# thedeemon/jsplayer

Measured on AMD Instinct MI355X. Metric: decoded Mpixels/sec at 1920x1080 (MSVideo1 + ScreenPressor), 1/2/4/8 GPUs, higher is better.
Workload: dtype u8

## Files before the change

jsplayer_amd/csrc/msv1.h:

```cpp
#pragma once
#include <cstddef>
#include <cstdint>
#include <vector>

#include <hip/hip_runtime.h>

namespace jsp {

constexpr uint32_t MSV1_DESC_SKIP = 0xFFFFFFFFu;
constexpr uint32_t MSV1_DESC_UNTOUCHED = 0xFFFFFFFEu;

struct Msv1FrameArgs {
    int32_t* dst;
    const int32_t* prev;
    uint32_t* signif;
    uint32_t stream_end;
    uint32_t desc_base;
    uint32_t cmp_row_lo;
    uint32_t pad;
};

constexpr uint32_t MSV1_FRAME_USES_PREV = 1u;
constexpr uint32_t MSV1_FRAME_NOOP = 2u;

// ... 30 lines not shown
constexpr uint32_t MSV1_INFO_END_MARKER = 1u;
constexpr uint32_t MSV1_INFO_S1 = 2u;
struct Msv1FrameInfo {
    uint32_t n_coded;
    uint32_t n_skip_codes;
    uint32_t total_blocks;
    uint32_t flags;
    uint32_t consumed;
    uint32_t pad[3];
};
uint32_t msv1_parse_tile_bytes();
uint32_t msv1_small_tile_bytes();
void msv1_launch_parse(const Msv1Geometry& geo, const uint8_t* d_stream, const Msv1ParseFrame* d_frames, int nframes,
                       const uint32_t* d_tile_frame, int ntiles, int max_tiles_per_frame, uint32_t* d_tile_tab,
                       uint32_t* d_tile_entry, uint32_t* d_tile_block0, uint32_t* d_desc, Msv1FrameInfo* d_info,
                       int insignificant_blocks, hipStream_t stream);

constexpr uint32_t MSV1_TILE_SKIP = 1u;
struct alignas(16) Msv1TileRec {
    uint32_t byte0;
    uint32_t frame_end;
    uint32_t data_end;
    uint32_t k;
    uint32_t first_tile;
    uint32_t ntiles;
    uint32_t cmp_row_lo;
    uint32_t flags;
    int32_t* dst;
    const int32_t* prev;
    uint32_t* signif;
    uint64_t pad;
};
static_assert(sizeof(Msv1TileRec) == 64, "one record = 64 bytes");
constexpr size_t MSV1_AGG_PUBLISHED = 9;
constexpr size_t MSV1_AGG_LAB_CLOCKS = 8;
constexpr size_t MSV1_SYNC_BYTES = 2 * sizeof(uint32_t) + 64;

struct Msv1FusedBatch {
    const uint8_t* stream = nullptr;
    const Msv1TileRec* recs = nullptr;
    const int32_t* palette = nullptr;
    unsigned long long* agg = nullptr;
    uint32_t epoch = 0;
    uint32_t tile0 = 0;
    int ntiles = 0;
    uint32_t* fault = nullptr;
    uint32_t agg_tiles = 0;
};
void msv1_launch_fused_pixels(const Msv1Geometry& geo, const Msv1FusedBatch& batch, hipStream_t stream);
void msv1_launch_fused_tables(const Msv1Geometry& geo, const Msv1FusedBatch& batch, hipStream_t stream);

constexpr uint32_t MSV1_ASYNC_SHORT = 1u;
constexpr uint32_t MSV1_ASYNC_S1 = 2u;
constexpr uint32_t MSV1_ASYNC_END = 4u;
constexpr uint32_t MSV1_ASYNC_SKIPCODE = 8u;
constexpr uint32_t MSV1_ASYNC_STUCK = 16u;
struct Msv1AsyncInfo {
    uint32_t flags;
    uint32_t signif;
    uint32_t fault;
    uint32_t arrived;
    uint32_t finished;
    uint32_t verdict;
    uint32_t pad[2];
};
constexpr uint32_t MSV1_VERDICT_GO = 1u, MSV1_VERDICT_VETO = 2u;
constexpr uint32_t MSV1_LAB_DEAF = 0x80000000u;
// ... 51 lines not shown
```

jsplayer_amd/csrc/msv1_codec.cpp:

```cpp
#include <algorithm>
#include <atomic>
#include <memory>
#include <exception>
#include <thread>
#include <unordered_set>

#include "codec.h"
#include "msv1.h"
#include "msv1_seek.h"
#include <msv1_fused_hooks.h>

namespace jsp {
namespace {

inline uint32_t next_epoch(uint32_t& e) { if (++e == 0) ++e; return e; }

inline size_t agg_bytes(size_t tiles) { return sizeof(unsigned long long) * (MSV1_AGG_PUBLISHED + MSV1_AGG_LAB_CLOCKS) * std::max<size_t>(tiles, 1); }

inline Msv1TileRec tile_rec(uint32_t beg, uint32_t even_end, uint32_t data_end, uint32_t k, uint32_t tile_bytes, uint32_t first_tile, uint32_t ntiles,
                            int32_t* dst, const int32_t* prev, uint32_t* signif, uint32_t cmp_row_lo, uint32_t flags) {
    Msv1TileRec r{};
    r.byte0 = beg + k * tile_bytes;
    r.frame_end = even_end;
    r.data_end = data_end;
// ... 125 lines not shown
                          d_tile_tab.as<uint32_t>(), d_tile_entry.as<uint32_t>(), d_tile_block0.as<uint32_t>(), d_desc.as<uint32_t>(), d_info.as<Msv1FrameInfo>(),
                          insignificant_blocks, stream);
    }

    void decode(hipStream_t stream) override {
        if (nframes == 0) return;
        last_stream = stream;
        const bool replay = gpu_parse && decoded && needs_desc;
        const bool run_ahead = side != nullptr && gpu_parse && needs_desc && ntiles_emit > 0;
        if (replay) {
            if (run_ahead && ahead_valid) JSP_HIP(hipStreamWaitEvent(stream, ev_tables, 0));
            else launch_table_parse(cur_set, stream);
        }
        const uint32_t* tables = replay ? wide_tables(cur_set) : d_desc.as<const uint32_t>();
        if (run_ahead && decoded) {
            try {
                make_set(cur_set ^ 1, stream);
            } catch (const std::exception&) {
                (void)hipGetLastError();
                sets[cur_set ^ 1].drop();
                side = nullptr;
            }
        }
        if (run_ahead && decoded && side) {
            if (!ev_fork) JSP_HIP(hipEventCreateWithFlags(&ev_fork, hipEventDisableTiming));
            if (!ev_tables) JSP_HIP(hipEventCreateWithFlags(&ev_tables, hipEventDisableTiming));
            JSP_HIP(hipEventRecord(ev_fork, stream));
            JSP_HIP(hipStreamWaitEvent(side, ev_fork, 0));
            launch_table_parse(cur_set ^ 1, side);
            JSP_HIP(hipEventRecord(ev_tables, side));
        }
        launch_groups(tables, true, stream);
        if (any_fused || needs_desc)
            JSP_HIP(hipMemcpyAsync(h_fault.p, d_sync.p, sizeof(uint32_t), hipMemcpyDeviceToHost, stream));
        ++clock_launches;
        if (run_ahead && decoded && side) { cur_set ^= 1; ahead_valid = true; }
        decoded = true;
    }
    void plan_launches(const std::vector<jsp_frame_in>& frames, const StagePlan& plan) {
        const auto& attr = plan.attr;
        const int nf = nframes;
        int i = 0;
        while (i < nf) {
            if (attr[i].special) { groups.push_back({i, 1, attr[i].edge, false, false}); ++i; continue; }
            int j = i;
            bool any_dep = false;
            while (j < nf && !attr[j].special) { any_dep |= attr[j].dependent; ++j; }
            std::unordered_set<const void*> seen;
            if (any_dep && vec_ok) {
                bool edge = false;
                for (int k = i; k < j; ++k) edge |= attr[k].edge;
                groups.push_back({i, j - i, edge, true, false});
            } else {
                bool closed = true;
                for (int k = i; k < j; ++k) {
                    const bool writes = !attr[k].noop;
                    const bool fusable = gpu_parse && vec_ok && !attr[k].dependent && !attr[k].noop && !plan.h_pf[k].host_parsed;
                    if (attr[k].dependent || closed || (writes && seen.count(frames[k].dst)) || groups.back().fused != fusable) {
                        groups.push_back({k, 1, attr[k].edge, false, fusable});
                        seen.clear();
                        closed = attr[k].dependent;
                    } else {
                        groups.back().count++;
                    }
                    if (writes) seen.insert(frames[k].dst);
                }
            }
// ... 19 lines not shown
            uint64_t written = 0, prev_reads = 0, sbytes = 0;
            bool uses_prev = false, gpu_table = false;
            for (int k = g.first; k < g.first + g.count; ++k) {
                if (!plan.attr[k].noop) written += (uint64_t)geo.nblocks;
                uses_prev |= (h_frames[k].pad & MSV1_FRAME_USES_PREV) != 0;
                if (h_frames[k].pad & MSV1_FRAME_USES_PREV) prev_reads += (uint64_t)geo.nblocks;
                sbytes += plan.frame_stream[k];
                gpu_table |= gpu_parse && !plan.h_pf[k].host_parsed;
            }
            moved += sbytes + 64 * written;
            if (g.fused) {
                any_fused = true;
                note_kernel("msv1_fused_kernel");
            } else {
                needs_desc |= gpu_table;
                moved += table_bytes_per_frame * g.count +
                         64 * (g.temporal ? (uses_prev ? (uint64_t)geo.nblocks : 0) : prev_reads);
                note_kernel(g.temporal ? "msv1_blocks_temporal_kernel" : "msv1_blocks_kernel");
            }
            if (g.edge_compare) note_kernel("msv1_edge_compare_kernel");
        }
        if (needs_desc) {
            moved += info.stream_bytes + table_bytes_per_frame * nf;
            if (!any_fused) kernels = "msv1_fused_kernel" + (kernels.empty() ? std::string() : " + " + kernels);
        }
        info.moved_bytes = moved;
        info.kernel_launches = groups.size() + (needs_desc ? 1 : 0);
    }

    void build_tile_records(const std::vector<jsp_frame_in>& frames, const StagePlan& plan, bool scrub_tables, hipStream_t stream) {
        if (!any_fused && !needs_desc) return;
        d_agg.reserve(agg_bytes((size_t)ntiles));
        d_sync.reserve(MSV1_SYNC_BYTES);
        h_fault.reserve(sizeof(uint32_t));
        *h_fault.as<uint32_t>() = 0;
        epoch = 0;
        build_pixel_records(plan, stream);
        if (needs_desc) build_table_records(frames, plan, scrub_tables, stream);
        JSP_HIP(hipMemsetAsync(d_agg.p, 0, agg_bytes((size_t)ntiles), stream));
        JSP_HIP(hipMemsetAsync(d_sync.p, 0, MSV1_SYNC_BYTES, stream));
    }
    void build_pixel_records(const StagePlan& plan, hipStream_t stream) {
        const int nf = nframes;
        const Msv1ParseFrame* h_pf = plan.h_pf;
        const auto* h_frames = this->h_frames.as<const Msv1FrameArgs>();
        h_recs.reserve(sizeof(Msv1TileRec) * (size_t)std::max(ntiles, 1));
        d_recs.reserve(sizeof(Msv1TileRec) * (size_t)std::max(ntiles, 1));
        auto* recs = h_recs.as<Msv1TileRec>();
        std::vector<uint32_t> nt16((size_t)nf);
        for (int i = 0; i < nf; ++i) {
            nt16[i] = h_pf[i].ntiles;
            for (uint32_t k = 0; k < h_pf[i].ntiles; ++k)
                recs[h_pf[i].first_tile + k] = tile_rec(h_pf[i].beg, h_pf[i].end, geo.bits == 16 ? h_pf[i].end : h_frames[i].stream_end, k, msv1_parse_tile_bytes(),
                                                        h_pf[i].first_tile, h_pf[i].ntiles, h_frames[i].dst, h_frames[i].prev, h_frames[i].signif,
                                                        h_frames[i].cmp_row_lo, h_pf[i].host_parsed ? MSV1_TILE_SKIP : 0u);
        }
        auto tile_major = [&](int f0, int f1) {
            if (f1 - f0 < 2) return;
            const uint32_t t0 = h_pf[f0].first_tile, t1 = h_pf[f1 - 1].first_tile + h_pf[f1 - 1].ntiles;
            const std::vector<Msv1TileRec> tmp(recs + t0, recs + t1);
            uint32_t o = t0;
            staggered_tile_order(f0, f1, nt16, MSV1_TILE_STAGGER, [&](int i, uint32_t k) { recs[o++] = tmp[h_pf[i].first_tile - t0 + k]; });
        };
        for (const auto& g : groups)
            if (g.fused) tile_major(g.first, g.first + g.count);
        JSP_HIP(hipMemcpyAsync(d_recs.p, recs, sizeof(Msv1TileRec) * (size_t)ntiles, hipMemcpyHostToDevice, stream));
    }
    void build_table_records(const std::vector<jsp_frame_in>& frames, const StagePlan& plan, bool scrub_tables, hipStream_t stream) {
        const int nf = nframes;
        const Msv1ParseFrame* h_pf = plan.h_pf;
        const auto* h_frames = this->h_frames.as<const Msv1FrameArgs>();
        const size_t nblk = (size_t)std::max(geo.nblocks, 1);
        const uint32_t tile8 = msv1_small_tile_bytes();
// ... 27 lines not shown
    }

    void launch_groups(const uint32_t* tables, bool fused, hipStream_t stream) {
        if (need_signif) JSP_HIP(hipMemsetAsync(d_signif.p, 0, sizeof(uint32_t) * nframes, stream));
        const auto* frames = d_frames.as<const Msv1FrameArgs>();
        for (const Group& g : groups) {
            if (g.fused && fused) {
                const auto* pf = h_pframes.as<const Msv1ParseFrame>();
                const uint32_t tile0 = pf[g.first].first_tile;
                const Msv1ParseFrame& last = pf[g.first + g.count - 1];
                msv1_launch_fused_pixels(geo, fused_batch(d_recs, d_agg, ntiles, tile0, (int)(last.first_tile + last.ntiles - tile0)), stream);
            } else if (g.temporal) {
                msv1_launch_blocks_temporal(geo, d_stream.as<const uint8_t>(), tables, frames + g.first, g.count, d_palette, stream);
            } else {
                msv1_launch_blocks(geo, d_stream.as<const uint8_t>(), tables, frames + g.first, g.count, d_palette, vec_ok, stream);
            }
            if (g.edge_compare) msv1_launch_edge_compare(geo, frames + g.first, g.count, stream);
        }
        JSP_HIP(hipGetLastError());
        if (need_signif) JSP_HIP(hipMemcpyAsync(h_signif.p, d_signif.p, sizeof(uint32_t) * nframes, hipMemcpyDeviceToHost, stream));
    }
    int clock_launches = 0;
    void after_sync() override {
        if (kFusedClocks && clock_launches) {
            std::vector<unsigned long long> c((size_t)ntiles * MSV1_AGG_LAB_CLOCKS);
            unsigned long long* dev = d_agg.as<unsigned long long>() + (size_t)ntiles * MSV1_AGG_PUBLISHED;
            JSP_HIP(hipMemcpy(c.data(), dev, c.size() * 8, hipMemcpyDeviceToHost));
            JSP_HIP(hipMemset(dev, 0, c.size() * 8));
            unsigned long long h[8] = {0, 0, 0, 0, 0, 0, 0, 0};
            for (size_t i = 0; i < c.size(); ++i) h[i & 7] += c[i];
            const unsigned long long n = (unsigned long long)ntiles * clock_launches;
            std::fprintf(stderr, "fused clocks per tile (cycles; %d tiles x %d launches): load %llu | tables+trees %llu | look-back %llu | down %llu | replay %llu | decode %llu\n",
                         ntiles, clock_launches, h[0] / n, h[1] / n, h[2] / n, h[3] / n, h[4] / n, h[5] / n);
        }
        clock_launches = 0;
        if ((any_fused || needs_desc) && (*h_fault.as<const uint32_t>() || inject_fault)) {
            inject_fault = false;
            ++fallback_runs;
            if (fallback_total) ++*fallback_total;
            note_kernel("msv1_parse_tiles (look-back fallback)");
            *h_fault.as<uint32_t>() = 0;
            hipStream_t stream = last_stream;
            quiesce_side();
            JSP_HIP(hipMemsetAsync(d_sync.p, 0, MSV1_SYNC_BYTES, stream));
            launch_parse(stream);
            launch_groups(d_desc.as<const uint32_t>(), false, stream);
            JSP_HIP(hipStreamSynchronize(stream));
        }
    }
    hipStream_t last_stream = nullptr;
    bool inject_fault = false;
    int fallback_runs = 0;
    std::shared_ptr<std::atomic<long long>> fallback_total;
};

struct Msv1AsyncStaged : jsp_staged {
    Msv1AsyncStaged() { verdict_pending = true; }
    Msv1Geometry geo{};
    Msv1AsyncShared shared;
    int ntiles = 0;
    size_t nbytes = 0;
    bool have_prev = false, compare = false, key = false;
    bool key_compare = false;
    DeviceBuffer d_stream, d_meta, d_agg;
    PinnedBuffer h_stream, h_meta, h_info;
    uint32_t epoch = 0;
    size_t agg_tiles = 0;
    bool merged = false;
    bool deaf = false;
    Msv1TileRec rec{};
    DeviceBuffer d_report;
    uint32_t want = 0;
    const uint8_t* src_dev = nullptr;
    hipEvent_t uploaded = nullptr;
    bool dma = false;
    bool stale_before = false;
    const void* full_dev_before = nullptr;
    size_t full_dev_bytes_before = 0;
    ~Msv1AsyncStaged() override { if (uploaded) (void)hipEventDestroy(uploaded); }

    Msv1AsyncInfo* d_info() const {
        if (merged) return d_report.as<Msv1AsyncInfo>();
        return reinterpret_cast<Msv1AsyncInfo*>(d_meta.as<uint8_t>() + sizeof(Msv1TileRec) * (size_t)ntiles);
    }
    uint32_t bad_mask() const { return MSV1_ASYNC_SHORT | MSV1_ASYNC_END | MSV1_ASYNC_STUCK | (have_prev ? 0u : MSV1_ASYNC_SKIPCODE) | (deaf ? MSV1_LAB_DEAF : 0u); }
    Msv1GroupFrame group_frame(hipStream_t stream) {
// ... 17 lines not shown
    void decode(hipStream_t stream) override {
        if (merged) { decode_with({}, stream); return; }
        Msv1FusedPass pass;
        pass.stream = d_stream.as<const uint8_t>();  pass.recs = d_meta.as<const Msv1TileRec>();  pass.ntiles = ntiles;
        pass.agg = d_agg.as<unsigned long long>();   pass.info = d_info();  pass.bad_mask = bad_mask();  pass.shared = shared;
        pass.epoch = next_epoch(epoch);
        msv1_launch_fused_scout(geo, pass, stream);
        pass.epoch = next_epoch(epoch);
        msv1_launch_fused_decode(geo, pass, stream);
        JSP_HIP(hipGetLastError());
        JSP_HIP(hipMemcpyAsync(h_info.p, pass.info, sizeof(Msv1AsyncInfo), hipMemcpyDeviceToHost, stream));
        decoded = true;
    }
};

std::atomic<int> g_async_streams{0};
constexpr int kDmaStreams = 3;

struct Msv1Codec : jsp_codec {
    Msv1Geometry geo{};
    size_t size_of_just_skips = 0;
    int insignificant_blocks = 0;
    bool insign_lines_set = false;
    int insign_lines = 0;
    std::vector<uint8_t> block_changes;
    std::vector<uint8_t> palette_bytes;
    int32_t palette[256];
    DeviceBuffer d_palette;
    bool opt_gpu_parse = true;
    bool opt_scrub_tables = false;
    bool opt_inject_fault = false;
    bool opt_inject_deaf = false;
    std::shared_ptr<std::atomic<long long>> lookback_fallbacks = std::make_shared<std::atomic<long long>>(0);
    long long counter(const char* name) override {
        if (std::strcmp(name, "prefetched_frames") == 0) return prefetched_frames;
        if (std::strcmp(name, "paired_frames") == 0) return paired_frames;
        if (std::strcmp(name, "host_parsed_frames") == 0) return host_parsed_frames;
        if (std::strcmp(name, "msv1_block_changes") == 0) {
            std::vector<uint8_t> rows;
            try {
                if (!msv1_block_changes_now(this, rows)) return -1;
            } catch (const std::exception&) {
                return -1;
            }
            long long m = 0;
            for (size_t r = 0; r < rows.size() && r < 62; ++r) m |= (long long)(rows[r] != 0) << r;
            return m;
        }
        return std::strcmp(name, "lookback_fallbacks") == 0 ? lookback_fallbacks->load() : -1;
    }
    bool opt_async_merged = true, opt_async_dma = true, opt_async_auto = true;
    bool counted_async = false;
    hipStream_t up_stream = nullptr;
    struct UpRange {
        const uint8_t* host = nullptr;
        size_t bytes = 0, skew = 0;
        DeviceBuffer dev;
        hipEvent_t up = nullptr, last_use = nullptr;
        bool waited = false;
        hipStream_t waited_on = nullptr;
        bool used = false;
    };
    static constexpr int kRanges = 4;
    UpRange ranges[kRanges];
    unsigned range_next = 0;
    hipStream_t prefetch_stream = nullptr;
    long long prefetched_frames = 0;
    long long host_parsed_frames = 0;
    int prefetch(const void* host, size_t n) override {
        if (!host || n == 0) {
            for (UpRange& r : ranges) { r.host = nullptr; r.bytes = 0; }
            return 0;
        }
        if (!opt_gpu_parse) return 0;
        launch_held();
        UpRange& r = ranges[range_next++ % kRanges];
        r.host = nullptr;
        r.bytes = 0;
        if (!prefetch_stream) JSP_HIP(hipStreamCreateWithFlags(&prefetch_stream, hipStreamNonBlocking));
        if (!r.up) {
            JSP_HIP(hipEventCreateWithFlags(&r.up, hipEventDisableTiming));
// ... 207 lines not shown
            block_changes_stale = false;
        }
        msv1_parse(geo, src, n, prev_dev != nullptr, size_of_just_skips, insignificant_blocks, base, desc,
                   block_changes, pr);
    }

    struct Prescan { bool sync_path, changes; };
    Prescan prescan(const uint8_t* src, size_t n) const {
        if (n < 2 || (geo.bits == 16 && n < size_of_just_skips)) return {true, false};
        long covered = 0;
        for (size_t si = 0; si + 1 < n && covered < geo.nblocks; si += 2) {
            const unsigned a = src[si], b = src[si + 1];
            if (geo.bits == 8 && a == 0 && b == 0) return {true, false};
            if ((b & 0xFC) != 0x84) return {false, true};
            const long cnt = (long)(((b - 0x84) << 8) + a);
            if (cnt == 0) return {true, false};
            covered += cnt;
        }
        return {covered < geo.nblocks, false};
    }

    bool sync_staging(const jsp_frame_in& f, const Prescan& ps) const {
        const bool aligned = (X & 3) == 0 && !(reinterpret_cast<uintptr_t>(f.dst) & 15) && !(reinterpret_cast<uintptr_t>(prev_dev) & 15);
        return !opt_gpu_parse || !aligned || (Y & 3) || ps.sync_path || geo.nblocks <= 0 || geo.nblocks >= (1 << 20) ||
               f.n + msv1_parse_tile_bytes() > 0xFFFFFFF0u || (geo.bits == 8 && !d_palette.p);
    }
    bool async_settle_first(const jsp_frame_in& f) override { return sync_staging(f, prescan(f.src, f.n)); }
    bool sync_through_async() const override { return opt_gpu_parse; }

    void reserve_async_buffers(Msv1AsyncStaged& st, int nt, size_t tile_bytes) {
        st.d_stream.reserve((size_t)nt * tile_bytes + 64);
        st.h_info.reserve(sizeof(Msv1AsyncInfo));
        if ((size_t)nt > st.agg_tiles) {
            st.d_agg.reserve(sizeof(unsigned long long) * 9 * (size_t)nt);
            st.agg_tiles = st.d_agg.cap / (sizeof(unsigned long long) * 9);
            JSP_HIP(hipMemsetAsync(st.d_agg.p, 0, st.d_agg.cap, stream));
        }
        if (st.merged && !st.d_report.p) {
            st.d_report.reserve(sizeof(Msv1AsyncInfo));
            JSP_HIP(hipMemsetAsync(st.d_report.p, 0, sizeof(Msv1AsyncInfo), stream));
            st.want = 0;
        }
        if (!st.merged) {
            const size_t meta_bytes = sizeof(Msv1TileRec) * (size_t)nt + sizeof(Msv1AsyncInfo);
            st.d_meta.reserve(meta_bytes);
            st.h_meta.reserve(meta_bytes);
        }
    }

    struct FrameBytes { const void* up; const uint8_t* up_dev; UpRange* range; };
    FrameBytes frame_bytes(const jsp_frame_in& f, Msv1AsyncStaged& st) {
        hipPointerAttribute_t attr{};
        UpRange* range = range_of(f.src, f.n);
        if (range) {
            if (!range->waited || range->waited_on != stream) {
                JSP_HIP(hipStreamWaitEvent(stream, range->up, 0));
                range->waited = true;
                range->waited_on = stream;
            }
            range->used = true;
            ++prefetched_frames;
            return {f.src, range->dev.as<const uint8_t>() + range->skew + (f.src - range->host), range};
        }
        if (hipPointerGetAttributes(&attr, f.src) == hipSuccess && attr.type == hipMemoryTypeHost)
            return {f.src, static_cast<const uint8_t*>(attr.devicePointer ? attr.devicePointer : f.src), nullptr};
        (void)hipGetLastError();
        st.h_stream.reserve(f.n + 16);
        std::memcpy(st.h_stream.p, f.src, f.n);
// ... 150 lines not shown
        st->build_tile_records(frames, plan, opt_scrub_tables, stream);
        st->info.host_stage_ms = now_ms() - t0 - plan.gpu_parse_ms;
        final_uploads(*st, plan);
        st->info.h2d_ms = plan.h2d_ms;
        st->info.device_parse_ms = plan.gpu_parse_ms;
        guard.release();
        return st;
    }

    void upload(void* d, const void* h, size_t bytes) {
        if (bytes) JSP_HIP(hipMemcpyAsync(d, h, bytes, hipMemcpyHostToDevice, stream));
    }

    void reset_batch(Msv1Staged& st, int nf) {
        st.quiesce_side();
        st.drop_sets();
        st.side = nullptr;
        if (opt_parse_ahead) {
            if (!side_stream) JSP_HIP(hipStreamCreateWithFlags(&side_stream, hipStreamNonBlocking));
            st.side = side_stream;
        }
        st.geo = geo;
        st.nframes = nf;
        st.decoded = false;
        st.groups.clear();
        st.status.assign(nf, JSP_ZERO_STATE);
        st.adopted.assign(nf, 0);
        st.significant.assign(nf, 0);
        st.info = jsp_staged_info{};
        st.why.clear();
        st.insignificant_blocks = insignificant_blocks;
        st.inject_fault = opt_inject_fault;
        st.fallback_total = lookback_fallbacks;
        st.gpu_parse = opt_gpu_parse && geo.nblocks > 0 && geo.nblocks < (1 << 20);
        if (geo.bits == 8 && !d_palette.p) {
            d_palette.reserve(sizeof palette);
            JSP_HIP(hipMemcpy(d_palette.p, palette, sizeof palette, hipMemcpyHostToDevice));
        }
        st.d_palette = d_palette.as<const int32_t>();
    }

    void lay_out_and_gather(const std::vector<jsp_frame_in>& frames, Msv1Staged& st, StagePlan& plan) {
        const int nf = (int)frames.size();
        const size_t nblk = (size_t)std::max(geo.nblocks, 1);
        plan.beg.resize(nf);
        const size_t frame_align = st.gpu_parse ? (size_t)msv1_parse_tile_bytes() : 16;
        for (int i = 0; i < nf; ++i) {
            plan.beg[i] = plan.total_stream;
            plan.total_stream += (frames[i].n + frame_align - 1) / frame_align * frame_align;
        }
        if (plan.total_stream + 64 > 0xFFFFFFF0u) throw std::runtime_error("batch stream exceeds 4 GiB");
        plan.in_pinned.assign(nf, 0);
        size_t gather_bytes = 0;
        for (int i = 0; i < nf; ++i) {
            if (st.gpu_parse && frames[i].n >= 4096) {
                hipPointerAttribute_t attr{};
                if (hipPointerGetAttributes(&attr, frames[i].src) == hipSuccess && attr.type == hipMemoryTypeHost) plan.in_pinned[i] = 1;
                else (void)hipGetLastError();
            }
            if (!plan.in_pinned[i]) gather_bytes += frames[i].n;
        }
        if (gather_bytes || !st.gpu_parse) st.h_stream.reserve(plan.total_stream + 64);
        if (!st.gpu_parse) st.h_desc.reserve(sizeof(uint32_t) * nblk * std::max(nf, 1));
        st.h_frames.reserve(sizeof(Msv1FrameArgs) * std::max(nf, 1));
        st.d_signif.reserve(sizeof(uint32_t) * std::max(nf, 1));
        st.h_signif.reserve(sizeof(uint32_t) * std::max(nf, 1));
// ... 280 lines not shown
```

jsplayer_amd/csrc/msv1_fused_hooks.h:

```cpp
#pragma once

#define JSP_BATCH_LS 32
#define JSP_FUSED_ALIGN 1
#define JSP_FUSED_VMCNT 4
#define JSP_FUSED_WAVES 4
#define JSP_FUSED_WAVES_TABLES 4
#define JSP_FUSED_LDS_PAD 0
#define JSP_CLOCK_BEGIN() do { } while (0)
#define JSP_CLOCK(k) do { } while (0)
constexpr bool kFusedClocks = false;
```

jsplayer_amd/csrc/msv1_lanes.h:

```cpp
#pragma once
#include <cstdint>

#if defined(JSP_LANES_HOST)
#define JSP_LANE_FN inline
#else
#define JSP_LANE_FN __device__ __forceinline__
#endif

namespace jsp {
namespace lanes {

#if defined(JSP_LANES_HOST)
inline uint32_t perm_b32(uint32_t s0, uint32_t s1, uint32_t sel) {
    const uint64_t in = ((uint64_t)s0 << 32) | s1;
    uint32_t out = 0;
    for (int k = 0; k < 4; ++k) {
        const uint32_t s = (sel >> (8 * k)) & 0xFFu;
        uint32_t b;
        if (s >= 13) b = 0xFF;
        else if (s == 12) b = 0;
        else if (s >= 8) b = ((in >> (8 * (2 * (s - 8) + 1) + 7)) & 1u) ? 0xFFu : 0u;
        else b = (uint32_t)(in >> (8 * s)) & 0xFFu;
        out |= b << (8 * k);
    }
// ... 121 lines not shown
            const uint32_t mz = sign_mask_c<S>(fZ);                                                          \
            add = (special_count16<LS>(w, m, S) & mz) | (16u & ~mz);                                         \
        }                                                                                                    \
        const uint32_t v = sat_add(nx, add);                                                                 \
        dw[8] = dw[7]; dw[7] = dw[6]; dw[6] = dw[5]; dw[5] = dw[4]; dw[4] = dw[3]; dw[3] = dw[2]; dw[2] = dw[1]; dw[1] = dw[0]; \
        dw[0] = v;                                                                                           \
        if (((S) & (JSP_LANE_FENCE_EVERY - 1)) == 0) JSP_LANE_SCHED_FENCE(dw[0], fM, fL, fZ);                \
    }
    if (LS == 32) {
        JSP_LANE_STEP(31) JSP_LANE_STEP(30) JSP_LANE_STEP(29) JSP_LANE_STEP(28) JSP_LANE_STEP(27) JSP_LANE_STEP(26) JSP_LANE_STEP(25) JSP_LANE_STEP(24)
        JSP_LANE_STEP(23) JSP_LANE_STEP(22) JSP_LANE_STEP(21) JSP_LANE_STEP(20) JSP_LANE_STEP(19) JSP_LANE_STEP(18) JSP_LANE_STEP(17) JSP_LANE_STEP(16)
    }
    JSP_LANE_STEP(15) JSP_LANE_STEP(14) JSP_LANE_STEP(13) JSP_LANE_STEP(12) JSP_LANE_STEP(11) JSP_LANE_STEP(10) JSP_LANE_STEP(9) JSP_LANE_STEP(8)
    JSP_LANE_STEP(7) JSP_LANE_STEP(6) JSP_LANE_STEP(5) JSP_LANE_STEP(4) JSP_LANE_STEP(3) JSP_LANE_STEP(2) JSP_LANE_STEP(1) JSP_LANE_STEP(0)
#undef JSP_LANE_STEP
#pragma unroll
    for (int e = 0; e < 9; ++e) tab[e] = dw[e];
}

template <int BITS, int LS>
JSP_LANE_FN uint32_t visited(const Masks& m, uint32_t entry_slot) {
    constexpr int MIDL = BITS == 16 ? 3 : 2, LONGL = BITS == 16 ? 9 : 5;
    constexpr uint32_t ALL = LS == 32 ? 0xFFFFFFFFu : ((1u << (LS & 31)) - 1u);
    const uint32_t S = ~(m.M | m.L);
    uint32_t V = (1u << entry_slot) & ALL;
    for (;;) {
        const uint32_t V2 = (V | ((V & S) << 1) | ((V & m.M) << MIDL) | ((V & m.L) << LONGL)) & ALL;
        if (V2 == V) break;
        V = V2;
    }
    return V;
}

}
}
```

jsplayer_amd/csrc/msv1_parse_kernels.hip:

```cpp
#include <algorithm>
#include <cstdio>
#include <cstdlib>
#include <vector>
#include "msv1.h"
#include "msv1_lanes.h"
#include "msv1_decode.h"
#include <msv1_fused_hooks.h>

namespace jsp {
namespace {

constexpr int PWG = 256;
constexpr int LSLOTS = JSP_BATCH_LS;
constexpr int TSLOTS = PWG * LSLOTS;
constexpr uint32_t BSAT = (1u << 28) - 1;

__device__ __forceinline__ uint32_t pack(uint32_t exit_slot, uint32_t blocks) { return exit_slot | (blocks << 4); }
__device__ __forceinline__ uint32_t add_blocks(uint32_t v, uint32_t n) {
    const uint32_t b = (v >> 4) + n;
    return (v & 15u) | ((b > BSAT ? BSAT : b) << 4);
}
__device__ __forceinline__ uint32_t compose(uint32_t a, const uint32_t* tb) {
    return add_blocks(tb[a & 15u], a >> 4);
}
// ... 234 lines not shown
                const uint32_t nb = blk + (c >> 8);
                blk = nb > BSAT ? BSAT : nb;
                if (blk >= nblocks) consumed = p0 + 2u * s + 2u * (c & 15u) - fr.beg;
            }
            pos += c & 15u;
        }
    }
    if (staged) {
        __syncthreads();
        for (uint32_t i = threadIdx.x; i < span; i += PWG) gdesc[tb0 + i] = stage[i];
    }
    const unsigned long long any = __ballot(ncoded | nskipcodes | flags | s1 | consumed);
    if (any) {
        uint32_t a = ncoded, b = nskipcodes, c2 = flags | (s1 ? MSV1_INFO_S1 : 0u);
#pragma unroll
        for (int o = 32; o > 0; o >>= 1) {
            a += __shfl_xor((int)a, o);
            b += __shfl_xor((int)b, o);
            c2 |= (uint32_t)__shfl_xor((int)c2, o);
        }
        if ((threadIdx.x & 63) == 0) {
            if (a) atomicAdd(&info[f].n_coded, a);
            if (b) atomicAdd(&info[f].n_skip_codes, b);
            if (c2) atomicOr(&info[f].flags, c2);
        }
        if (consumed) info[f].consumed = consumed;
    }
}


constexpr uint32_t F_SKIP = 0xFFFFu;
constexpr uint32_t F_NONE = 0xFFFEu;
constexpr int LOOKBACK_SPIN_LIMIT = 1 << 18;
constexpr int VERDICT_SPIN_LIMIT = 1 << 15;

__device__ __forceinline__ uint32_t wave_or(uint32_t v) {
    v |= (uint32_t)__builtin_amdgcn_update_dpp(0, (int)v, 0xB1, 0xF, 0xF, true);
    v |= (uint32_t)__builtin_amdgcn_update_dpp(0, (int)v, 0x4E, 0xF, 0xF, true);
    v |= (uint32_t)__builtin_amdgcn_update_dpp(0, (int)v, 0x141, 0xF, 0xF, true);
    v |= (uint32_t)__builtin_amdgcn_update_dpp(0, (int)v, 0x140, 0xF, 0xF, true);
    return (uint32_t)__builtin_amdgcn_readlane((int)v, 0) | (uint32_t)__builtin_amdgcn_readlane((int)v, 16) |
           (uint32_t)__builtin_amdgcn_readlane((int)v, 32) | (uint32_t)__builtin_amdgcn_readlane((int)v, 48);
}

template <int BITS, int MODE, int LS>
__global__ __launch_bounds__(PWG, MODE == 4 ? JSP_FUSED_WAVES_TABLES : JSP_FUSED_WAVES) void msv1_fused_kernel(const uint8_t* __restrict__ stream_p,
                                                            const Msv1TileRec* __restrict__ recs,
                                                            const int32_t* __restrict__ palette,
                                                            unsigned long long* __restrict__ agg_p, uint32_t epoch_p,
                                                            uint32_t tile0, uint32_t* __restrict__ fault_p,
                                                            uint32_t nblocks, int nbx, int X,
                                                            Msv1AsyncInfo* __restrict__ info_p, uint32_t s1_first_block,
                                                            uint32_t bad_mask_p, uint32_t* __restrict__ poison,
                                                            Msv1TileRec one_rec_p, Msv1AsyncInfo* __restrict__ host_info_p, uint32_t want_p,
                                                            uint8_t* __restrict__ keep_p, Msv1Riders riders) {
    uint32_t ride = 0;
    if (MODE == 3)
        for (uint32_t q = 0; q < riders.count; ++q) ride = blockIdx.x >= riders.f[q].first_wg ? q + 1u : ride;
    const bool rider = MODE == 3 && ride != 0u;
    const Msv1Rider& rd = riders.f[rider ? ride - 1u : 0u];
    const uint32_t bid = rider ? blockIdx.x - rd.first_wg : blockIdx.x;
    const uint8_t* __restrict__ stream = rider ? rd.stream : stream_p;
    unsigned long long* __restrict__ agg = rider ? rd.agg : agg_p;
    const uint32_t epoch = rider ? rd.epoch : epoch_p;
    Msv1AsyncInfo* __restrict__ info = rider ? rd.info : info_p;
    uint32_t* __restrict__ fault = rider ? &rd.info->fault : fault_p;
    const uint32_t bad_mask = rider ? rd.bad_mask : bad_mask_p;
    Msv1AsyncInfo* __restrict__ host_info = rider ? rd.host_info : host_info_p;
    const uint32_t want = rider ? rd.want : want_p;
    uint8_t* __restrict__ keep = rider ? rd.keep : keep_p;
    const Msv1AsyncInfo* info_before = ride >= 2u ? riders.f[ride - 2u].info : info_p;
    const uint32_t want_before = ride >= 2u ? riders.f[ride - 2u].want : want_p;
    const uint32_t epoch_before = ride >= 2u ? riders.f[ride - 2u].epoch : epoch_p;
    constexpr bool INFO = MODE == 1 || MODE == 3;
    constexpr bool USES_PREV = MODE != 0;
    constexpr int TSLOTS = PWG * LS;
    constexpr int FSTAGE = 4096;
    constexpr uint32_t TILE_BYTES = TSLOTS * 2;
    constexpr int LSLOTS = LS;
    constexpr int LBW = LS == 32 ? 3 : 5, LOOKBACK_BATCH = LBW * PWG / 9, LOOKBACK_SEGS = LBW * 7 / 3;
    constexpr bool PREFIX = MODE == 0 || MODE == 4;
    constexpr int BYTES_W = TSLOTS * 2 / 4 + 8, TAB_W = PWG * 9 + 16, ENTER_W = PREFIX ? 4 : LOOKBACK_BATCH * 9 + 4;
    static_assert(TAB_W * 2 >= FSTAGE, "staging window must fit in the tables' space");
    __shared__ __align__(16) uint32_t arena[BYTES_W + TAB_W + ENTER_W + JSP_FUSED_LDS_PAD];
    __shared__ uint32_t s_pal[BITS == 8 ? 256 : 1];
    __shared__ uint32_t s_entry, s_root[16], s_seg[PREFIX ? 1 : LOOKBACK_SEGS][9];
    __shared__ uint32_t s_grp[PWG / 64][7][16], s_wav[PWG / 64][16];
    uint8_t* lds_bytes = reinterpret_cast<uint8_t*>(arena);
    uint32_t* tabs = arena + BYTES_W;
    uint32_t* enter = arena + BYTES_W + TAB_W;
    uint16_t* stage = reinterpret_cast<uint16_t*>(arena + BYTES_W);
    const int tid = threadIdx.x, lane = tid & 63, wave = tid >> 6;
    auto wave_sync = [] { asm volatile("s_waitcnt lgkmcnt(0)" ::: "memory"); __builtin_amdgcn_wave_barrier(); };
    JSP_CLOCK_BEGIN();
    Msv1TileRec r = MODE == 3 ? (rider ? rd.rec : one_rec_p) : recs[tile0 + blockIdx.x];
    if (MODE == 3) r.k = bid;
    const uint32_t t = PREFIX ? r.first_tile + r.k : tile0 + bid;
    if (MODE != 3 && (r.flags & MSV1_TILE_SKIP)) return;
    auto arrive = [&] { __threadfence(); atomicAdd(&info->arrived, 1u); };
    auto finish = [&] {
        __threadfence();
        if (atomicAdd(&info->finished, 1u) + 1u == want) {
            __threadfence();
            host_info->flags = __hip_atomic_load(&info->flags, __ATOMIC_RELAXED, __HIP_MEMORY_SCOPE_AGENT);
            host_info->signif = __hip_atomic_load(&info->signif, __ATOMIC_RELAXED, __HIP_MEMORY_SCOPE_AGENT);
            host_info->fault = __hip_atomic_load(&info->fault, __ATOMIC_RELAXED, __HIP_MEMORY_SCOPE_AGENT);
            __hip_atomic_store(&info->flags, 0u, __ATOMIC_RELAXED, __HIP_MEMORY_SCOPE_AGENT);
            __hip_atomic_store(&info->signif, 0u, __ATOMIC_RELAXED, __HIP_MEMORY_SCOPE_AGENT);
            __hip_atomic_store(&info->fault, 0u, __ATOMIC_RELAXED, __HIP_MEMORY_SCOPE_AGENT);
            __hip_atomic_store(&info->verdict, 0u, __ATOMIC_RELAXED, __HIP_MEMORY_SCOPE_AGENT);
        }
    };
    if (MODE == 3) {
        if (__hip_atomic_load(poison, __ATOMIC_RELAXED, __HIP_MEMORY_SCOPE_AGENT)) {
            if (threadIdx.x == 0) {
                __hip_atomic_store(&info->pad[0], epoch, __ATOMIC_RELAXED, __HIP_MEMORY_SCOPE_AGENT);
                arrive();
                finish();
            }
            return;
        }
    }
    if (MODE == 2) {
        const bool bad = (info->flags & bad_mask) != 0u;
        if (bad && blockIdx.x == 0 && threadIdx.x == 0) atomicOr(poison, 1u);
        if (bad || __hip_atomic_load(poison, __ATOMIC_RELAXED, __HIP_MEMORY_SCOPE_AGENT)) return;
    }
    if (BITS == 8) s_pal[tid] = (uint32_t)palette[tid];
    const uint32_t k = r.k;
    const uint32_t tile_byte0 = PREFIX ? r.byte0 : t * TILE_BYTES;
    const uint32_t data_end = r.data_end;

    const uint32_t nlook = k < (uint32_t)LOOKBACK_BATCH ? k : (uint32_t)LOOKBACK_BATCH;
    const uint32_t look0 = k - nlook;
    unsigned long long lv[LBW];
#pragma unroll
    for (int q = 0; q < LBW; ++q) lv[q] = 0ull;
    if (PREFIX) {
        if (tid == 0 && k) lv[0] = __hip_atomic_load(agg + (size_t)(t - 1u) * 9u, __ATOMIC_RELAXED, __HIP_MEMORY_SCOPE_AGENT);
    } else {
        const unsigned long long* look_src = agg + (size_t)(r.first_tile + look0) * 9u;
#pragma unroll
        for (int q = 0; q < LBW; ++q)
            if ((uint32_t)(tid + q * PWG) < nlook * 9u)
                lv[q] = __hip_atomic_load(look_src + tid + q * PWG, __ATOMIC_RELAXED, __HIP_MEMORY_SCOPE_AGENT);
    }

    {
        constexpr int NLOAD = (BYTES_W * 4 + PWG * 16 - 1) / (PWG * 16);
        uint4 v[NLOAD];
#pragma unroll
        for (int q = 0; q < NLOAD; ++q) {
            const uint32_t o = tid * 16u + (uint32_t)q * (PWG * 16u), at = tile_byte0 + o;
            v[q] = make_uint4(0, 0, 0, 0);
            if (o < (uint32_t)BYTES_W * 4u && at < data_end && !(MODE == 3 && data_end - at < 16u))
                v[q] = *reinterpret_cast<const uint4*>(stream + at);
        }
#pragma unroll
        for (int q = 0; q < NLOAD; ++q) {
            const uint32_t o = tid * 16u + (uint32_t)q * (PWG * 16u), at = tile_byte0 + o;
            if (o >= (uint32_t)BYTES_W * 4u) continue;
            if (at < data_end) {
                const uint32_t nvalid = data_end - at;
                if (nvalid < 16u) {
                    if (MODE == 3) {
                        uint32_t wds[4] = {0, 0, 0, 0};
                        for (uint32_t i = 0; i < nvalid; ++i) wds[i >> 2] |= (uint32_t)stream[at + i] << (8u * (i & 3u));
                        v[q] = make_uint4(wds[0], wds[1], wds[2], wds[3]);
                    }
                    auto keep_bytes = [&](uint32_t word, uint32_t first) -> uint32_t {
                        if (nvalid >= first + 4u) return word;
                        if (nvalid <= first) return 0u;
// ... 30 lines not shown
            uint32_t v = (uint32_t)e1;
#pragma unroll
            for (int q = 0; q < 10; ++q) {
                if (q < cnt) {
                    v = lanes::sat_add(row[v & 15u], v & ~15u);
                    row[e1] = v;
                    row += 9;
                }
            }
            s_grp[wave][g1][e1] = v;
        }
        wave_sync();
        if (lane < 9) {
            uint32_t v = (uint32_t)lane;
#pragma unroll
            for (int g = 0; g < 7; ++g) {
                v = lanes::sat_add(s_grp[wave][g][v & 15u], v & ~15u);
                s_grp[wave][g][lane] = v;
            }
            s_wav[wave][lane] = v;
        }
    }
    __syncthreads();
    JSP_CLOCK(1);
    if (tid < 9) {
        uint32_t v = (uint32_t)tid;
#pragma unroll
        for (int u = 0; u < PWG / 64; ++u) {
            v = lanes::sat_add(s_wav[u][v & 15u], v & ~15u);
            s_wav[u][tid] = v;
        }
        s_root[tid] = v;
        const uint32_t pv = (v >> 4) >= BSAT ? (BSAT << 4) : v;
        if (!PREFIX && k + 1u < r.ntiles)
            __hip_atomic_store(agg + (size_t)t * 9u + tid, ((unsigned long long)epoch << 32) | pv, __ATOMIC_RELAXED, __HIP_MEMORY_SCOPE_AGENT);
    }
    if (PREFIX) {
        if (tid == 0) {
            uint32_t ent = 0;
            bool ok = true;
            if (k) {
                for (int spin = 0; (uint32_t)(lv[0] >> 32) != epoch; ++spin) {
                    if (spin > LOOKBACK_SPIN_LIMIT) { ok = false; break; }
                    __builtin_amdgcn_s_sleep(8);
                    lv[0] = __hip_atomic_load(agg + (size_t)(t - 1u) * 9u, __ATOMIC_RELAXED, __HIP_MEMORY_SCOPE_AGENT);
                }
                ent = (uint32_t)lv[0];
            }
            if (ok) {
                const uint32_t after = lanes::sat_add(s_root[ent & 15u], ent & ~15u);
                if (k + 1u < r.ntiles)
                    __hip_atomic_store(agg + (size_t)t * 9u, ((unsigned long long)epoch << 32) | ((after >> 4) >= BSAT ? (BSAT << 4) : after),
                                       __ATOMIC_RELAXED, __HIP_MEMORY_SCOPE_AGENT);
            } else {
                atomicOr(fault, 1u);
            }
            s_entry = ok ? ent : 0xFFFFFFFFu;
        }
        __syncthreads();
        if (s_entry == 0xFFFFFFFFu) return;
    } else {
        uint32_t e = 0, blocks = 0;
        for (uint32_t j0 = 0; j0 < k; j0 += LOOKBACK_BATCH) {
            const bool last = j0 + LOOKBACK_BATCH >= k;
            const uint32_t b0 = last ? look0 : j0, nj = last ? nlook : (uint32_t)LOOKBACK_BATCH;
            const unsigned long long* src = agg + (size_t)(r.first_tile + b0) * 9u;
            unsigned long long v[LBW];
            bool have = true;
#pragma unroll
            for (int q = 0; q < LBW; ++q) {
                const bool wanted = (uint32_t)(tid + q * PWG) < nj * 9u;
                v[q] = last ? lv[q] : (wanted ? __hip_atomic_load(src + tid + q * PWG, __ATOMIC_RELAXED, __HIP_MEMORY_SCOPE_AGENT) : 0ull);
            }
#pragma unroll
            for (int q = 0; q < LBW; ++q) {
                const bool wanted = (uint32_t)(tid + q * PWG) < nj * 9u;
                have &= !wanted || (uint32_t)(v[q] >> 32) == epoch;
            }
            for (int spin = 0; !__syncthreads_and(have); ++spin) {
                if (spin > LOOKBACK_SPIN_LIMIT) {
                    if (tid == 0) {
                        atomicOr(fault, 1u);
                        if (MODE >= 1 && MODE <= 3) atomicOr(&info->flags, MSV1_ASYNC_STUCK);
                        if (MODE == 2 || MODE == 3) atomicOr(poison, 1u);
                        if (MODE == 3) { arrive(); finish(); }
                    }
                    return;
                }
                __builtin_amdgcn_s_sleep(8);
                have = true;
// ... 356 lines not shown
```

Before: 1.419 million.

## Use decoupled look-back over published tile tables in prefix parse mode

In prefix mode each tile now publishes its 9-entry transition table next to its inclusive prefix word. When the predecessor's prefix is not yet ready, one wave polls up to six predecessor tiles and folds their published tables onto the nearest available prefix, so it no longer waits on a strict serial chain. The change also counts tiles resolved through tables and reads that counter back on the host. Cost: wider agg records, extra atomic stores per tile, and a larger shared-memory enter window.

```diff
diff --git a/jsplayer_amd/csrc/msv1.h b/jsplayer_amd/csrc/msv1.h
--- a/jsplayer_amd/csrc/msv1.h
+++ b/jsplayer_amd/csrc/msv1.h
@@ -86,7 +86,9 @@
     uint64_t pad;
 };
 static_assert(sizeof(Msv1TileRec) == 64, "one record = 64 bytes");
-constexpr size_t MSV1_AGG_PUBLISHED = 9;
+constexpr size_t MSV1_AGG_TABLE_WORDS = 9;
+constexpr size_t MSV1_AGG_PUBLISHED = 16;
+constexpr size_t MSV1_AGG_PREFIX_WORD = 9;
 constexpr size_t MSV1_AGG_LAB_CLOCKS = 8;
 constexpr size_t MSV1_SYNC_BYTES = 2 * sizeof(uint32_t) + 64;
 
diff --git a/jsplayer_amd/csrc/msv1_codec.cpp b/jsplayer_amd/csrc/msv1_codec.cpp
--- a/jsplayer_amd/csrc/msv1_codec.cpp
+++ b/jsplayer_amd/csrc/msv1_codec.cpp
@@ -181,7 +181,7 @@
         }
         launch_groups(tables, true, stream);
         if (any_fused || needs_desc)
-            JSP_HIP(hipMemcpyAsync(h_fault.p, d_sync.p, sizeof(uint32_t), hipMemcpyDeviceToHost, stream));
+            JSP_HIP(hipMemcpyAsync(h_fault.p, d_sync.p, 2 * sizeof(uint32_t), hipMemcpyDeviceToHost, stream));
         ++clock_launches;
         if (run_ahead && decoded && side) { cur_set ^= 1; ahead_valid = true; }
         decoded = true;
@@ -267,13 +267,13 @@
         if (!any_fused && !needs_desc) return;
         d_agg.reserve(agg_bytes((size_t)ntiles));
         d_sync.reserve(MSV1_SYNC_BYTES);
-        h_fault.reserve(sizeof(uint32_t));
-        *h_fault.as<uint32_t>() = 0;
+        h_fault.reserve(2 * sizeof(uint32_t));
+        h_fault.as<uint32_t>()[0] = h_fault.as<uint32_t>()[1] = 0;
         epoch = 0;
         build_pixel_records(plan, stream);
         if (needs_desc) build_table_records(frames, plan, scrub_tables, stream);
         JSP_HIP(hipMemsetAsync(d_agg.p, 0, agg_bytes((size_t)ntiles), stream));
-        JSP_HIP(hipMemsetAsync(d_sync.p, 0, MSV1_SYNC_BYTES, stream));
+        clear_sync_words(stream);
     }
     void build_pixel_records(const StagePlan& plan, hipStream_t stream) {
         const int nf = nframes;
@@ -367,17 +367,23 @@
             const unsigned long long n = (unsigned long long)ntiles * clock_launches;
             std::fprintf(stderr, "fused clocks per tile (cycles; %d tiles x %d launches): load %llu | tables+trees %llu | look-back %llu | down %llu | replay %llu | decode %llu\n",
                          ntiles, clock_launches, h[0] / n, h[1] / n, h[2] / n, h[3] / n, h[4] / n, h[5] / n);
+            jsp_lab_clock_table(c.data(), (size_t)ntiles, clock_launches);
         }
         clock_launches = 0;
+        if (any_fused || needs_desc) {
+            const uint32_t now = h_fault.as<const uint32_t>()[1];
+            if (aggregate_total) *aggregate_total += (long long)(uint32_t)(now - aggregate_seen);
+            aggregate_seen = now;
+        }
         if ((any_fused || needs_desc) && (*h_fault.as<const uint32_t>() || inject_fault)) {
             inject_fault = false;
             ++fallback_runs;
             if (fallback_total) ++*fallback_total;
             note_kernel("msv1_parse_tiles (look-back fallback)");
-            *h_fault.as<uint32_t>() = 0;
+            h_fault.as<uint32_t>()[0] = h_fault.as<uint32_t>()[1] = 0;
             hipStream_t stream = last_stream;
             quiesce_side();
-            JSP_HIP(hipMemsetAsync(d_sync.p, 0, MSV1_SYNC_BYTES, stream));
+            clear_sync_words(stream);
             launch_parse(stream);
             launch_groups(d_desc.as<const uint32_t>(), false, stream);
             JSP_HIP(hipStreamSynchronize(stream));
@@ -387,6 +393,12 @@
     bool inject_fault = false;
     int fallback_runs = 0;
     std::shared_ptr<std::atomic<long long>> fallback_total;
+    std::shared_ptr<std::atomic<long long>> aggregate_total;
+    uint32_t aggregate_seen = 0;
+    void clear_sync_words(hipStream_t stream) {
+        JSP_HIP(hipMemsetAsync(d_sync.p, 0, MSV1_SYNC_BYTES, stream));
+        aggregate_seen = 0;
+    }
 };
 
 struct Msv1AsyncStaged : jsp_staged {
@@ -470,6 +482,7 @@
     bool opt_inject_fault = false;
     bool opt_inject_deaf = false;
     std::shared_ptr<std::atomic<long long>> lookback_fallbacks = std::make_shared<std::atomic<long long>>(0);
+    std::shared_ptr<std::atomic<long long>> lookback_aggregate_tiles = std::make_shared<std::atomic<long long>>(0);
     long long counter(const char* name) override {
         if (std::strcmp(name, "prefetched_frames") == 0) return prefetched_frames;
         if (std::strcmp(name, "paired_frames") == 0) return paired_frames;
@@ -485,6 +498,7 @@
             for (size_t r = 0; r < rows.size() && r < 62; ++r) m |= (long long)(rows[r] != 0) << r;
             return m;
         }
+        if (std::strcmp(name, "lookback_aggregate_tiles") == 0) return lookback_aggregate_tiles->load();
         return std::strcmp(name, "lookback_fallbacks") == 0 ? lookback_fallbacks->load() : -1;
     }
     bool opt_async_merged = true, opt_async_dma = true, opt_async_auto = true;
@@ -758,8 +772,8 @@
         st.d_stream.reserve((size_t)nt * tile_bytes + 64);
         st.h_info.reserve(sizeof(Msv1AsyncInfo));
         if ((size_t)nt > st.agg_tiles) {
-            st.d_agg.reserve(sizeof(unsigned long long) * 9 * (size_t)nt);
-            st.agg_tiles = st.d_agg.cap / (sizeof(unsigned long long) * 9);
+            st.d_agg.reserve(sizeof(unsigned long long) * MSV1_AGG_TABLE_WORDS * (size_t)nt);
+            st.agg_tiles = st.d_agg.cap / (sizeof(unsigned long long) * MSV1_AGG_TABLE_WORDS);
             JSP_HIP(hipMemsetAsync(st.d_agg.p, 0, st.d_agg.cap, stream));
         }
         if (st.merged && !st.d_report.p) {
@@ -976,6 +990,7 @@
         st.insignificant_blocks = insignificant_blocks;
         st.inject_fault = opt_inject_fault;
         st.fallback_total = lookback_fallbacks;
+        st.aggregate_total = lookback_aggregate_tiles;
         st.gpu_parse = opt_gpu_parse && geo.nblocks > 0 && geo.nblocks < (1 << 20);
         if (geo.bits == 8 && !d_palette.p) {
             d_palette.reserve(sizeof palette);
diff --git a/jsplayer_amd/csrc/msv1_fused_hooks.h b/jsplayer_amd/csrc/msv1_fused_hooks.h
--- a/jsplayer_amd/csrc/msv1_fused_hooks.h
+++ b/jsplayer_amd/csrc/msv1_fused_hooks.h
@@ -9,3 +9,4 @@
 #define JSP_CLOCK_BEGIN() do { } while (0)
 #define JSP_CLOCK(k) do { } while (0)
 constexpr bool kFusedClocks = false;
+inline void jsp_lab_clock_table(const unsigned long long*, size_t, int) {}
diff --git a/jsplayer_amd/csrc/msv1_lanes.h b/jsplayer_amd/csrc/msv1_lanes.h
--- a/jsplayer_amd/csrc/msv1_lanes.h
+++ b/jsplayer_amd/csrc/msv1_lanes.h
@@ -177,5 +177,14 @@
     return V;
 }
 
+constexpr uint32_t PUBLISHED_SAT = (1u << 28) - 1;
+JSP_LANE_FN uint32_t published(uint32_t v) { return (v >> 4) >= PUBLISHED_SAT ? PUBLISHED_SAT << 4 : v; }
+
+JSP_LANE_FN uint32_t fold_prefix(uint32_t prefix, const uint32_t* tables, uint32_t n, uint32_t stride) {
+    uint32_t v = prefix;
+    for (uint32_t j = n; j-- > 0;) v = published(sat_add(tables[j * stride + (v & 15u)], v & ~15u));
+    return v;
+}
+
 }
 }
diff --git a/jsplayer_amd/csrc/msv1_parse_kernels.hip b/jsplayer_amd/csrc/msv1_parse_kernels.hip
--- a/jsplayer_amd/csrc/msv1_parse_kernels.hip
+++ b/jsplayer_amd/csrc/msv1_parse_kernels.hip
@@ -290,6 +290,9 @@
 constexpr uint32_t F_SKIP = 0xFFFFu;
 constexpr uint32_t F_NONE = 0xFFFEu;
 constexpr int LOOKBACK_SPIN_LIMIT = 1 << 18;
+constexpr int LOOKBACK_NEAR = 6, LOOKBACK_NEAR_WORDS = (int)MSV1_AGG_PREFIX_WORD + 1;
+static_assert(LOOKBACK_NEAR * LOOKBACK_NEAR_WORDS <= 64, "the miss path's words are fetched by the lanes of one wave");
+static_assert(BSAT == lanes::PUBLISHED_SAT, "one saturation bound for everything published");
 constexpr int VERDICT_SPIN_LIMIT = 1 << 15;
 
 __device__ __forceinline__ uint32_t wave_or(uint32_t v) {
@@ -338,7 +341,7 @@
     constexpr int LSLOTS = LS;
     constexpr int LBW = LS == 32 ? 3 : 5, LOOKBACK_BATCH = LBW * PWG / 9, LOOKBACK_SEGS = LBW * 7 / 3;
     constexpr bool PREFIX = MODE == 0 || MODE == 4;
-    constexpr int BYTES_W = TSLOTS * 2 / 4 + 8, TAB_W = PWG * 9 + 16, ENTER_W = PREFIX ? 4 : LOOKBACK_BATCH * 9 + 4;
+    constexpr int BYTES_W = TSLOTS * 2 / 4 + 8, TAB_W = PWG * 9 + 16, ENTER_W = PREFIX ? LOOKBACK_NEAR * LOOKBACK_NEAR_WORDS + 4 : LOOKBACK_BATCH * 9 + 4;
     static_assert(TAB_W * 2 >= FSTAGE, "staging window must fit in the tables' space");
     __shared__ __align__(16) uint32_t arena[BYTES_W + TAB_W + ENTER_W + JSP_FUSED_LDS_PAD];
     __shared__ uint32_t s_pal[BITS == 8 ? 256 : 1];
@@ -395,7 +398,8 @@
 #pragma unroll
     for (int q = 0; q < LBW; ++q) lv[q] = 0ull;
     if (PREFIX) {
-        if (tid == 0 && k) lv[0] = __hip_atomic_load(agg + (size_t)(t - 1u) * 9u, __ATOMIC_RELAXED, __HIP_MEMORY_SCOPE_AGENT);
+        if (tid == 0 && k)
+            lv[0] = __hip_atomic_load(agg + (size_t)(t - 1u) * MSV1_AGG_PUBLISHED + MSV1_AGG_PREFIX_WORD, __ATOMIC_RELAXED, __HIP_MEMORY_SCOPE_AGENT);
     } else {
         const unsigned long long* look_src = agg + (size_t)(r.first_tile + look0) * 9u;
 #pragma unroll
@@ -492,30 +496,57 @@
         }
         s_root[tid] = v;
         const uint32_t pv = (v >> 4) >= BSAT ? (BSAT << 4) : v;
-        if (!PREFIX && k + 1u < r.ntiles)
-            __hip_atomic_store(agg + (size_t)t * 9u + tid, ((unsigned long long)epoch << 32) | pv, __ATOMIC_RELAXED, __HIP_MEMORY_SCOPE_AGENT);
+        if ((PREFIX ? k != 0u : true) && k + 1u < r.ntiles)
+            __hip_atomic_store(agg + (size_t)t * (PREFIX ? MSV1_AGG_PUBLISHED : MSV1_AGG_TABLE_WORDS) + tid, ((unsigned long long)epoch << 32) | pv,
+                               __ATOMIC_RELAXED, __HIP_MEMORY_SCOPE_AGENT);
     }
     if (PREFIX) {
-        if (tid == 0) {
-            uint32_t ent = 0;
+        if (wave == 0) {
+            uint32_t ent = (uint32_t)lv[0], through = 0;
             bool ok = true;
-            if (k) {
-                for (int spin = 0; (uint32_t)(lv[0] >> 32) != epoch; ++spin) {
+            if (k && (uint32_t)__builtin_amdgcn_readfirstlane((int)(uint32_t)(lv[0] >> 32)) != epoch) {
+                constexpr uint32_t NW = LOOKBACK_NEAR_WORDS;
+                const uint32_t nd = k < (uint32_t)LOOKBACK_NEAR ? k : (uint32_t)LOOKBACK_NEAR;
+                const uint32_t back = (uint32_t)lane / NW, word = (uint32_t)lane - back * NW;
+                const bool wanted = (uint32_t)lane < nd * NW;
+                const unsigned long long* src = agg + (size_t)(t - 1u - (wanted ? back : 0u)) * MSV1_AGG_PUBLISHED + word;
+                unsigned long long v = 0ull;
+                bool present = false;
+                uint32_t m = 0;
+                for (int spin = 0;; ++spin) {
+                    if (wanted && !present) {
+                        v = __hip_atomic_load(src, __ATOMIC_RELAXED, __HIP_MEMORY_SCOPE_AGENT);
+                        present = (uint32_t)(v >> 32) == epoch;
+                    }
+                    const unsigned long long have = __ballot(present);
+                    for (uint32_t q = 0; q < nd && !m; ++q) {
+                        const uint32_t bits = (uint32_t)(have >> (q * NW)) & ((1u << NW) - 1u);
+                        if (bits >> MSV1_AGG_PREFIX_WORD) m = q + 1u;
+                        else if ((bits & 0x1FFu) != 0x1FFu) break;
+                    }
+                    if (m) break;
                     if (spin > LOOKBACK_SPIN_LIMIT) { ok = false; break; }
                     __builtin_amdgcn_s_sleep(8);
-                    lv[0] = __hip_atomic_load(agg + (size_t)(t - 1u) * 9u, __ATOMIC_RELAXED, __HIP_MEMORY_SCOPE_AGENT);
-                }
-                ent = (uint32_t)lv[0];
-            }
-            if (ok) {
-                const uint32_t after = lanes::sat_add(s_root[ent & 15u], ent & ~15u);
-                if (k + 1u < r.ntiles)
-                    __hip_atomic_store(agg + (size_t)t * 9u, ((unsigned long long)epoch << 32) | ((after >> 4) >= BSAT ? (BSAT << 4) : after),
-                                       __ATOMIC_RELAXED, __HIP_MEMORY_SCOPE_AGENT);
-            } else {
-                atomicOr(fault, 1u);
-            }
-            s_entry = ok ? ent : 0xFFFFFFFFu;
+                }
+                if (ok) {
+                    if (wanted) enter[lane] = (uint32_t)v;
+                    wave_sync();
+                    ent = lanes::fold_prefix(enter[(m - 1u) * NW + MSV1_AGG_PREFIX_WORD], enter, m - 1u, NW);
+                    through = m - 1u;
+                }
+            }
+            if (lane == 0) {
+                if (ok) {
+                    const uint32_t after = lanes::sat_add(s_root[ent & 15u], ent & ~15u);
+                    if (k + 1u < r.ntiles)
+                        __hip_atomic_store(agg + (size_t)t * MSV1_AGG_PUBLISHED + MSV1_AGG_PREFIX_WORD, ((unsigned long long)epoch << 32) | lanes::published(after),
+                                           __ATOMIC_RELAXED, __HIP_MEMORY_SCOPE_AGENT);
+                    if (through) atomicAdd(fault + 1, 1u);
+                } else {
+                    atomicOr(fault, 1u);
+                }
+                s_entry = ok ? ent : 0xFFFFFFFFu;
+            }
         }
         __syncthreads();
         if (s_entry == 0xFFFFFFFFu) return;
```

New measurement: 1.374 million. 0.968x the previous value.
